# Superjie13/StereoTracking

Hardware: AMD Instinct MI355X
Metric: stereo frame-pairs/sec @1280x720 D=192 (higher is better)
Workload: dtype f32; 1 GPU; configs[1]: batch=8 synthetic 1280x720 stereo pairs per GPU, D=192, full YOLOX-s two-branch backbone+PAFPN+head, cost volume at 1/4 res (48 levels) + 2 3x3 aggregation convs + soft-argmin, decode+NMS, per-box depth; global_batch=8, inflight_contexts=4, distinct_input_batches=4, gpu_max_hw_queues=4, hip_force_dev_kernarg=1, parallelism=single process, no process group (no collective in the step), collectives_issued=0, tuning_plan=configs/tuning/mi355x.json, max_det=1000, detections_overflow=False

## Files before the change

include/stereotrack.h:

```cpp
#ifndef STEREOTRACK_H_
#define STEREOTRACK_H_

#include <stddef.h>
#include <stdint.h>

#ifdef __cplusplus
extern "C" {
#endif

#define ST_VERSION 430

enum {
  ST_OK = 0,
  ST_ERR_INVALID = -1,
  ST_ERR_HIP = -2,
  ST_ERR_STATE = -3,
  ST_ERR_WORKSPACE = -4,
  ST_ERR_NOTFOUND = -5
};

typedef void* st_stream_t;

int st_version(void);
const char* st_last_error(void);

typedef struct StConvDesc {
  const float* in_dev;
  int N, Hi, Wi, Cin, in_ld, in_off;
  const float* wgt_dev;
  const float* bias_dev;
  int Cout, KH, KW, stride, pad;
  float* out1_dev;
  int out1_ld, out1_off, split;
  float* out2_dev;
  int out2_ld, out2_off;
  float* up_dev;
  int up_ld, up_off;
  const float* res_dev;
  int res_ld, res_off;
  float post_scale;
  int act;
  const float* wgt_wino_dev;
} StConvDesc;

int st_conv2d_nhwc(const StConvDesc* d, st_stream_t stream);
int st_conv2d_nhwc_variant(const StConvDesc* d, st_stream_t stream, int variant);
size_t st_wino_packed_floats(int Cout, int Cin);
int st_wino_pack_weights(const float* packed_wgt_host, int Cout, int Cin, float* out_host);
int st_conv3x3_wino_group(const StConvDesc* descs, int n, st_stream_t stream);

int st_conv1x1_chain(const StConvDesc* a, const StConvDesc* b, st_stream_t stream);
size_t st_front_frag_floats(int Cout, int Cin);
int st_front_pack_frags(const float* packed_wgt_host, int Cout, int Cin, float* out_host);
int st_conv3x3s2_csp_front(const StConvDesc* a, const StConvDesc* ms, const StConvDesc* c1, const float* frag_ms_dev,
                           const float* frag_c1_dev, st_stream_t stream);
size_t st_csp_tail_frag_floats(void);
int st_csp_tail_pack_frags(const float* packed_wgt_host, float* out_host);
int st_conv3x3_csp_tail(const StConvDesc* conv2, const StConvDesc* fin, const float* frag_fin_dev, st_stream_t stream);
size_t st_conv_packed_floats(int Cout, int Cin, int KH, int KW);
int st_conv_pack_weights(const float* w, const float* conv_bias,
                         const float* bn_gamma, const float* bn_beta,
                         const float* bn_mean, const float* bn_var,
                         double bn_eps, int Cout, int Cin, int KH, int KW,
                         float* wgt_out, float* bias_out);

int st_focus_pack(const float* img_nchw_dev, int N, int C, int H, int W,
                  float* out_nhwc_dev, st_stream_t stream);

size_t st_stem_packed_floats(int Cout);
int st_stem_pack_weights(const float* w, const float* conv_bias,
                         const float* bn_gamma, const float* bn_beta,
                         const float* bn_mean, const float* bn_var,
                         double bn_eps, int Cout, int used_planes, float* wgt_out, float* bias_out);
int st_stem_focus_conv(const float* img_nchw_dev, int N, int H, int W, int used_planes, const float* wgt_dev,
                       const float* bias_dev, int Cout, float* out_nhwc_dev, int out_ld, int out_off,
                       int act , st_stream_t stream);
int st_stem_focus_conv_u8(const unsigned char* const* frames_u8_dev_ptrs_host, int N, int h, int w, int H, int W,
                          float pad_value, const float* wgt_dev, const float* bias_dev, int Cout, float* out_dev,
                          int out_ld, int out_off, int act, st_stream_t stream);

int st_pack_raw_inputs(const unsigned char* img_u8_dev, const unsigned short* disp_u16_dev, int N, int h, int w,
                       int H, int W, float img_pad, float* img_out_dev, float* disp_postp_out_dev,
                       float* disp_mask_out_dev, st_stream_t stream);
int st_pack_raw_frames(const unsigned char* const* frames_u8_dev_ptrs_host, int N, int h, int w, int H, int W,
                       float img_pad, float* img_out_dev, st_stream_t stream);
int st_resize_planes(const void* in_dev, int P, int h, int w, int interleaved, void* out_dev, int h2, int w2,
                     int elem_bytes, int bilinear, st_stream_t stream);

int st_spp_pool(const float* x_dev, int x_ld, int x_off, int N, int H, int W, int C,
                float* out_dev, int out_ld, int out_off, st_stream_t stream);

typedef struct StDetector StDetector;

typedef struct StDetectorConfig {
  int struct_size;
  float widen_factor;
  float deepen_factor;
  int num_classes;
  int batch;
  int height, width;
  double bn_eps;
  int with_right_branch;
  int disp_planes_identical;
  int rgb_only;
} StDetectorConfig;

int st_detector_create(const StDetectorConfig* cfg, StDetector** out);
int st_detector_destroy(StDetector* det);

int st_detector_num_params(const StDetector* det);
int st_detector_param_info(const StDetector* det, int idx, char* name, int name_cap,
                           int64_t shape[4], int* ndim);
int st_detector_set_param(StDetector* det, const char* name, const float* host, int64_t numel);
int st_detector_finalize(StDetector* det);

size_t st_detector_workspace_bytes(const StDetector* det);
size_t st_detector_head_floats(const StDetector* det);
int st_detector_num_levels(const StDetector* det);
int st_detector_level_info(const StDetector* det, int level, int* h, int* w, int* stride,
                           size_t* float_offset);
int st_detector_forward(StDetector* det, const float* img_dev, const float* disp_dev,
                        void* workspace_dev, size_t workspace_bytes, st_stream_t stream,
                        float* head_out_dev);
double st_detector_macs(const StDetector* det);
int st_detector_forward_phase(StDetector* det, int phase, const float* img_dev,
                              const float* disp_dev, const float* right_dev, void* workspace_dev,
                              size_t workspace_bytes, st_stream_t stream, float* head_out_dev);
int st_detector_forward_phase0_raw(StDetector* det, const unsigned char* const* left_frames_host,
                                   const unsigned char* const* right_frames_host, int h, int w, float pad_value,
                                   void* workspace_dev, size_t workspace_bytes, st_stream_t stream);
int st_detector_forward_raw(StDetector* det, const unsigned char* const* img_frames_host, int h, int w,
                            float pad_value, const float* disp_dev, void* workspace_dev, size_t workspace_bytes,
                            st_stream_t stream, float* head_out_dev);
int st_detector_set_timing(StDetector* det, int enable);
int st_detector_num_ops(const StDetector* det);
int st_detector_op_times(StDetector* det, int cap, float* ms, int* kind, int* variant, double* macs,
                         int* phase);
int st_detector_op_desc(const StDetector* det, int i, char* buf, int cap);
int st_detector_op_owner(const StDetector* det, int cap, int* owner, int* variant);
int st_split_instances_available(void);
int st_detector_set_split(StDetector* det, int allow);
int st_detector_autotune(StDetector* det, void* workspace_dev, size_t workspace_bytes,
                         float* head_out_dev, st_stream_t stream, int reps);
const char* st_conv_variant_name(int id);
const char* st_conv_variant_signature(int id);
int st_detector_get_tuning(const StDetector* det, int* variants, int cap);
int st_detector_set_tuning(StDetector* det, const int* variants, int n);
int st_detector_tap(const StDetector* det, const char* name, const void* workspace_dev,
                    const float** ptr_dev, int* N, int* C, int* H, int* W, int* ld);
typedef struct StHeadPredLevel {
  const float* cls_dev;
  int cls_ld, cls_off;
  const float* reg_dev;
  int reg_ld, reg_off;
  const float* wgt_cls_dev;
  const float* bias_cls_dev;
  const float* wgt_reg_dev;
  const float* bias_reg_dev;
  float* out_dev;
  int M;
} StHeadPredLevel;
int st_head_pred(const StHeadPredLevel levels[3], int feat, int num_classes, st_stream_t stream);

typedef struct StDecodeDesc {
  int struct_size;
  int batch;
  int num_levels;
  int level_h[4], level_w[4], level_stride[4];
  size_t level_offset[4];
  float score_thr;
  float iou_thr;
  int max_det;
  float scale_x, scale_y;
// ... 449 lines not shown
```

stereotracking_amd/_lib.py:

```python
import ctypes as C
import os

import torch

_HERE = os.path.dirname(os.path.abspath(__file__))
LIB_PATH = os.path.join(_HERE, 'lib', 'libstereotrack_hip.so')

ST_OK = 0
_ERR_NAMES = {-1: 'ST_ERR_INVALID', -2: 'ST_ERR_HIP', -3: 'ST_ERR_STATE', -4: 'ST_ERR_WORKSPACE',
              -5: 'ST_ERR_NOTFOUND'}


class StError(RuntimeError):
    """A libstereotrack_hip call returned a non-zero status."""


class StConvDesc(C.Structure):
    _fields_ = [
        ('in_dev', C.c_void_p),
        ('N', C.c_int), ('Hi', C.c_int), ('Wi', C.c_int), ('Cin', C.c_int), ('in_ld', C.c_int), ('in_off', C.c_int),
        ('wgt_dev', C.c_void_p), ('bias_dev', C.c_void_p),
        ('Cout', C.c_int), ('KH', C.c_int), ('KW', C.c_int), ('stride', C.c_int), ('pad', C.c_int),
        ('out1_dev', C.c_void_p), ('out1_ld', C.c_int), ('out1_off', C.c_int), ('split', C.c_int),
        ('out2_dev', C.c_void_p), ('out2_ld', C.c_int), ('out2_off', C.c_int),
# ... 116 lines not shown
class StMotChallengeArgs(C.Structure):
    _fields_ = [(n, C.c_int) for n in ('struct_size', 'num_frames', 'num_gt', 'num_pred', 'max_frame_objects', 'do_preproc',
                                       'num_distractors')] + [('distractors', C.c_int * 8), ('num_ws_cells', C.c_longlong)] + \
        [(n, C.c_void_p) for n in ('gt_rows', 'pred_rows', 'frame_gt_off', 'frame_pred_off', 'frame_ws_off', 'ws')] + \
        [('ws_bytes', C.c_size_t)] + [(n, C.c_void_p) for n in ('gt_keep', 'pred_keep', 'status')]


class StTrackletArgs(C.Structure):
    _fields_ = [(n, C.c_int) for n in ('struct_size', 'num_rows', 'num_out_rows', 'num_tracks', 'first', 'count',
                                       'num_groups', 'max_rows')] + \
        [(n, C.c_void_p) for n in ('rows', 'row_out_off', 'row_gap', 'trk_out_off', 'trk_order', 'trk_len_scale', 'ws')] + \
        [('ws_bytes', C.c_size_t), ('out_rows', C.c_void_p), ('status', C.c_void_p), ('phase_ticks', C.c_void_p)]


class StAflinkArgs(C.Structure):
    _fields_ = [(n, C.c_int) for n in ('struct_size', 'num_sets', 'num_tracks', 'num_rows', 'capacity', 'first', 'count',
                                       'chunk')] + \
        [(n, C.c_double) for n in ('t_lo', 't_hi', 'spatial_thr')] + \
        [(n, C.c_void_p) for n in ('feat', 'trk_off', 'trk_set', 'set_off', 'ws_off', 'ws_x', 'header', 'cand', 'conf',
                                   'logits')]


class StStreamTick(C.Structure):
    _fields_ = [('struct_size', C.c_int), ('streams', C.c_int), ('chunk', C.c_int), ('num_chunks', C.c_int),
                ('max_dets', C.c_int), ('det_rows', C.c_int), ('stream_of_slot', C.c_void_p), ('frame_ids', C.c_void_p)]


class StHeadPredLevel(C.Structure):
    _fields_ = [('cls_dev', C.c_void_p), ('cls_ld', C.c_int), ('cls_off', C.c_int),
                ('reg_dev', C.c_void_p), ('reg_ld', C.c_int), ('reg_off', C.c_int),
                ('wgt_cls_dev', C.c_void_p), ('bias_cls_dev', C.c_void_p),
                ('wgt_reg_dev', C.c_void_p), ('bias_reg_dev', C.c_void_p),
                ('out_dev', C.c_void_p), ('M', C.c_int)]


class StDecodeDesc(C.Structure):
    _fields_ = [
        ('struct_size', C.c_int), ('batch', C.c_int), ('num_levels', C.c_int),
        ('level_h', C.c_int * 4), ('level_w', C.c_int * 4), ('level_stride', C.c_int * 4),
        ('level_offset', C.c_size_t * 4),
        ('score_thr', C.c_float), ('iou_thr', C.c_float), ('max_det', C.c_int),
        ('scale_x', C.c_float), ('scale_y', C.c_float), ('pad_left', C.c_float), ('pad_top', C.c_float),
        ('ori_w', C.c_float), ('ori_h', C.c_float), ('nms_mask_rows', C.c_int), ('num_classes', C.c_int),
        ('single_label', C.c_int),
    ]


_vp, _i, _f, _sz = C.c_void_p, C.c_int, C.c_float, C.c_size_t
_PROTOS = {
    'st_version': (C.c_int, []),
    'st_head_row_floats': (_i, [_i]),
    'st_png_unfilter': (_i, [_vp, _i, _i, _i, _vp]),
    'st_stem_focus_conv_u8': (_i, [_vp, _i, _i, _i, _i, _i, _f, _vp, _vp, _i, _vp, _i, _i, _i, _vp]),
    'st_detector_forward_raw': (_i, [_vp, _vp, _i, _i, _f, _vp, _vp, _sz, _vp, _vp]),
    'st_detector_forward_phase0_raw': (_i, [_vp, _vp, _vp, _i, _i, _f, _vp, _sz, _vp]),
    'st_pack_raw_frames': (_i, [_vp, _i, _i, _i, _i, _i, _f, _vp, _vp]),
    'st_resize_planes': (_i, [_vp, _i, _i, _i, _i, _vp, _i, _i, _i, _i, _vp]),
    'st_detector_set_split': (_i, [_vp, _i]),
    'st_split_instances_available': (_i, []),
    'st_volume_agg3d': (_i, [_vp, _vp, _i, _i, _i, _i, _vp, _f, _i, _vp]),
    'st_last_error': (C.c_char_p, []),
    'st_conv2d_nhwc': (_i, [C.POINTER(StConvDesc), _vp]),
    'st_conv2d_nhwc_variant': (_i, [C.POINTER(StConvDesc), _vp, _i]),
    'st_conv3x3_wino_group': (_i, [C.POINTER(StConvDesc), _i, _vp]),
    'st_head_pred': (_i, [C.POINTER(StHeadPredLevel), _i, _i, _vp]),
    'st_detector_op_owner': (_i, [_vp, _i, _vp, _vp]),
    'st_conv1x1_chain': (_i, [C.POINTER(StConvDesc), C.POINTER(StConvDesc), _vp]),
    'st_front_frag_floats': (_sz, [_i, _i]),
    'st_front_pack_frags': (_i, [_vp, _i, _i, _vp]),
    'st_conv3x3s2_csp_front': (_i, [C.POINTER(StConvDesc), C.POINTER(StConvDesc), C.POINTER(StConvDesc), _vp, _vp, _vp]),
    'st_csp_tail_frag_floats': (_sz, []),
    'st_csp_tail_pack_frags': (_i, [_vp, _vp]),
    'st_conv3x3_csp_tail': (_i, [C.POINTER(StConvDesc), C.POINTER(StConvDesc), _vp, _vp]),
    'st_conv_packed_floats': (_sz, [_i, _i, _i, _i]),
    'st_wino_packed_floats': (_sz, [_i, _i]),
    'st_wino_pack_weights': (_i, [_vp, _i, _i, _vp]),
    'st_conv_pack_weights': (_i, [_vp, _vp, _vp, _vp, _vp, _vp, C.c_double, _i, _i, _i, _i, _vp, _vp]),
    'st_focus_pack': (_i, [_vp, _i, _i, _i, _i, _vp, _vp]),
    'st_stem_packed_floats': (_sz, [_i]),
    'st_stem_pack_weights': (_i, [_vp, _vp, _vp, _vp, _vp, _vp, C.c_double, _i, _i, _vp, _vp]),
    'st_stem_focus_conv': (_i, [_vp, _i, _i, _i, _i, _vp, _vp, _i, _vp, _i, _i, _i, _vp]),
    'st_pack_raw_inputs': (_i, [_vp, _vp, _i, _i, _i, _i, _i, _f, _vp, _vp, _vp, _vp]),
    'st_spp_pool': (_i, [_vp, _i, _i, _i, _i, _i, _i, _vp, _i, _i, _vp]),
    'st_detector_create': (_i, [C.POINTER(StDetectorConfig), C.POINTER(_vp)]),
    'st_detector_destroy': (_i, [_vp]),
    'st_detector_num_params': (_i, [_vp]),
    'st_detector_param_info': (_i, [_vp, _i, C.c_char_p, _i, C.POINTER(C.c_int64), C.POINTER(_i)]),
    'st_detector_set_param': (_i, [_vp, C.c_char_p, _vp, C.c_int64]),
    'st_detector_finalize': (_i, [_vp]),
    'st_detector_workspace_bytes': (_sz, [_vp]),
    'st_detector_head_floats': (_sz, [_vp]),
    'st_detector_num_levels': (_i, [_vp]),
    'st_detector_level_info': (_i, [_vp, _i, C.POINTER(_i), C.POINTER(_i), C.POINTER(_i), C.POINTER(_sz)]),
    'st_detector_forward': (_i, [_vp, _vp, _vp, _vp, _sz, _vp, _vp]),
    'st_detector_forward_phase': (_i, [_vp, _i, _vp, _vp, _vp, _vp, _sz, _vp, _vp]),
    'st_detector_macs': (C.c_double, [_vp]),
    'st_detector_set_timing': (_i, [_vp, _i]),
    'st_detector_num_ops': (_i, [_vp]),
    'st_detector_op_times': (_i, [_vp, _i, _vp, _vp, _vp, _vp, _vp]),
    'st_detector_autotune': (_i, [_vp, _vp, _sz, _vp, _vp, _i]),
    'st_conv_variant_name': (C.c_char_p, [_i]),
    'st_conv_variant_signature': (C.c_char_p, [_i]),
    'st_detector_get_tuning': (_i, [_vp, _vp, _i]),
    'st_detector_set_tuning': (_i, [_vp, _vp, _i]),
    'st_detector_op_desc': (_i, [_vp, _i, C.c_char_p, _i]),
    'st_detector_tap': (_i, [_vp, C.c_char_p, _vp, C.POINTER(_vp), C.POINTER(_i), C.POINTER(_i),
                             C.POINTER(_i), C.POINTER(_i), C.POINTER(_i)]),
    'st_decode_nms_workspace_bytes': (_sz, [C.POINTER(StDecodeDesc)]),
    'st_lapjv_extended': (_i, [_vp, _i, _i, C.c_double, _vp, _vp]),
    'st_tracker_create': (_i, [C.POINTER(StTrackerConfig), C.POINTER(_vp)]),
    'st_tracker_destroy': (_i, [_vp]),
    'st_tracker_reset': (_i, [_vp]),
    'st_tracker_track': (_i, [_vp, _i, _vp, _i, _vp, _vp, _i, C.POINTER(_i)]),
    'st_tracker_track_records': (_i, [_vp, _vp, _vp, _i, _i, _i, _vp, _vp, _i, _vp]),
    'st_tracker_cmc_needed': (_i, [_vp, _i, _i]),
    'st_tracker_track_cmc': (_i, [_vp, _i, _vp, _i, _vp, _vp, _vp, _i, C.POINTER(_i)]),
    'st_tracker_track_records_cmc': (_i, [_vp, _vp, _vp, _i, _i, _i, _vp, _vp, C.POINTER(_i), _vp, _vp, _i, _vp,
                                          C.POINTER(_i)]),
    'st_cmc_num_levels': (_i, [_vp]),
    'st_cmc_workspace_bytes': (_sz, [_i]),
    'st_cmc_front_u8': (_i, [_vp, _i, _i, _i, _i, _i, _vp, _vp]),
    'st_cmc_front_f32': (_i, [_vp, _i, _i, _i, _i, _i, _vp, _vp]),
    'st_cmc_flow': (_i, [_vp, _vp, _i, _i, _vp, _sz, _vp, _vp, _vp]),
    'st_cmc_estimate': (_i, [_vp, _vp, _i, _i, _i, C.POINTER(StCmcParams), _vp, _sz, _vp, _vp, _vp, _vp]),
    'st_cmc_mesh_fit': (_i, [_vp, _i, _i, _i, C.POINTER(StCmcParams), _vp, _sz, _vp, _vp, _vp, _vp]),
    'st_cmc_fit': (_i, [_vp, _i, _i, C.c_float, C.c_float, _vp, _sz, _vp, _vp, _vp]),
    'st_cmc_ecc_plane_size': (_i, [_i, _i, _i, C.POINTER(_i), C.POINTER(_i)]),
    'st_cmc_ecc_workspace_bytes': (_sz, [_i, _i, _i]),
    'st_cmc_ecc_front_u8': (_i, [_vp, _i, _i, _i, _i, _i, _i, _vp, _vp]),
    'st_cmc_ecc_front_f32': (_i, [_vp, _i, _i, _i, _i, _i, _i, _vp, _vp]),
    'st_cmc_ecc_prepare': (_i, [_vp, _vp, _i, _i, _i, C.POINTER(StEccParams), _vp, _sz, _vp, _vp, _vp, _vp, _vp]),
    'st_cmc_ecc_step': (_i, [_vp, _vp, _i, _i, _i, C.POINTER(StEccParams), _vp, _vp, _sz, _vp, _vp]),
    'st_cmc_ecc_estimate': (_i, [_vp, _vp, _i, _i, _i, C.POINTER(StEccParams), _vp, _sz, _vp, _vp, _vp]),
    'st_sgbm_workspace_bytes': (_sz, [_i, _i, _i, _i]),
    'st_sgbm_u8': (_i, [_vp, _vp, _i, _i, _i, _i, _i, C.POINTER(StSgbmParams), _vp, _sz, _vp, _i, _i, _vp, _vp]),
    'st_sgbm_f32': (_i, [_vp, _vp, _i, _i, _i, _i, _i, C.POINTER(StSgbmParams), _vp, _sz, _vp, _vp, _vp]),
    'st_sgbm_match_f32': (_i, [_vp, _vp, _i, _i, _i, _i, _i, C.POINTER(StSgbmParams), _vp, _sz, _vp, _vp, _vp]),
    'st_sgbm_median': (_i, [_vp, _i, _i, _i, _vp, _vp]),
    'st_sgbm_speckle': (_i, [_vp, _i, _i, _i, _i, _i, _vp, _sz, _vp, _vp, _i, _i, _vp, _vp]),
    'st_tracker_num_tracks': (_i, [_vp]),
    'st_tracker_next_id': (C.c_longlong, [_vp]),
    'st_tracker_get_track': (_i, [_vp, _i, _vp, _vp, _vp, C.POINTER(_i), C.POINTER(_i), C.POINTER(_i)]),
    'st_tracker_get_states': (_i, [_vp, _vp, _i, _i, C.POINTER(_i), C.POINTER(C.c_longlong)]),
    'st_batched_tracker_get_states': (_i, [_vp, _vp, _i, _vp, _i, _i, C.POINTER(_i), C.POINTER(C.c_longlong),
                                           C.POINTER(_i), _vp]),
    'st_batched_tracker_create': (_i, [C.POINTER(StTrackerConfig), _i, _i, _i, C.POINTER(_vp)]),
    'st_batched_tracker_create_multi': (_i, [C.POINTER(StTrackerConfig), _i, _i, _i, C.POINTER(_vp)]),
    'st_batched_tracker_run': (_i, [_vp, _vp, _vp, _vp, _vp, _i, _i, _i, _i, _vp, _vp, _vp, _vp, _vp, _vp, _vp]),
    'st_batched_tracker_destroy': (_i, [_vp]),
    'st_batched_tracker_state_bytes': (_sz, [_vp]),
    'st_batched_tracker_scratch_bytes': (_sz, [_vp]),
    'st_batched_tracker_step': (_i, [_vp, _vp, _vp, _vp, _vp, _vp, _vp, _vp, _vp, _vp, _vp]),
    'st_decode_nms': (_i, [C.POINTER(StDecodeDesc), _vp, _vp, _sz, _vp, _vp, _vp, _vp, _vp, _vp]),
    'st_costvolume_softargmin': (_i, [_vp, _vp, _i, _i, _i, _i, _i, _i, _f, _vp, _vp, _vp]),
    'st_softargmin': (_i, [_vp, _i, _i, _i, _i, _f, _vp, _vp]),
    'st_disp_upsample_pack': (_i, [_vp, _i, _i, _i, _i, _i, _i, _i, _i, _vp, _vp]),
    'st_softargmin_right': (_i, [_vp, _i, _i, _i, _i, _f, _vp, _vp]),
    'st_lr_check_pack': (_i, [_vp, _vp, _i, _i, _i, _i, _i, _i, _i, _i, _f, _vp, _vp, _vp]),
    'st_feat_upsample': (_i, [_vp, _i, _i, _i, _i, _i, _i, _vp, _vp]),
    'st_costvolume_agg3d_supported': (_i, [_i, _i]),
    'st_costvolume_agg3d': (_i, [_vp, _vp, _i, _i, _i, _i, _i, _i, _vp, _f, _i, _vp, _vp]),
    'st_costvolume_agg3d_softargmin': (_i, [_vp, _vp, _i, _i, _i, _i, _i, _i, _vp, _f, _i, _f, _vp, _vp]),
    'st_box_depth_workspace_bytes': (_sz, [_i, _i, _i, _i]),
    'st_pack_records': (_i, [_vp, _vp, _vp, _vp, _vp, _vp, _vp, _vp, _i, _i, _i, _i, _vp, _vp]),
    'st_box_depth': (_i, [_vp, _sz, _i, _i, _i, _vp, _vp, _i, _f, _f, _vp, _sz, _vp, _vp, _vp, _vp]),
    'st_coco_max_gt': (_i, []),
# ... 76 lines not shown
```

stereotracking_amd/csrc/detector.cpp:

```cpp
#include <algorithm>
#include <cmath>
#include <cstring>
#include <map>
#include <memory>
#include <vector>

#include "st_common.h"

namespace st {

int conv2d_launch(const StConvDesc& d, hipStream_t stream, int force_variant, int* picked_variant);
bool pw_conv_applicable(const StConvDesc& d);
bool pw_chain_applicable(const StConvDesc& d, const StConvDesc& c);
bool dc_conv_applicable(const StConvDesc& d);
bool wino_conv_applicable(const StConvDesc& d);
bool wino_shape_ok(int Cin, int Cout);
bool wino_group_applicable(const StConvDesc* d, int n);
int wino_group_launch(const StConvDesc* d, int n, hipStream_t stream);
size_t wino_packed_floats(int Cout, int Cin);
int wino_pack_weights(const float* packed, int Cout, int Cin, float* out);
int pw_conv_launch(const StConvDesc& d, hipStream_t stream, const StConvDesc* chain);
bool pwr_conv_applicable(const StConvDesc& d);
bool pwr_chain_applicable(const StConvDesc& d, const StConvDesc& c);
int pwr_conv_launch(const StConvDesc& d, hipStream_t stream, const StConvDesc* chain);
bool front_fused_applicable(const StConvDesc& a, const StConvDesc& ms, const StConvDesc& c1);
int front_fused_launch(const StConvDesc& a, const StConvDesc& ms, const StConvDesc& c1, const float* frag_ms_dev,
                       const float* frag_c1_dev, hipStream_t stream);
size_t front_frag_floats(int Cout, int Cin);
int front_pack_frags(const float* packed, int Cout, int Cin, float* out);
bool csp_tail_applicable(const StConvDesc& c2, const StConvDesc& f);
int csp_tail_launch(const StConvDesc& c2, const StConvDesc& f, const float* frag_fin_dev, hipStream_t stream);
size_t csp_tail_frag_floats();
int csp_tail_pack_frags(const float* packed, float* out);
int conv_variant_count();
bool conv_variant_valid(int id, int cout);
const char* conv_variant_name(int id);
const char* conv_variant_signature(int id);
int focus_pack_launch(const float* img, int N, int C, int H, int W, float* out, hipStream_t stream);
int stem_focus_conv_launch(const float* in, int N, int H, int W, int used_planes, const float* wgt,
                           const float* bias, int Cout, float* out, int out_ld, int out_off, int act,
                           hipStream_t stream, const StemRawInput* raw);
int spp_pool_launch(const float* x, int x_ld, int x_off, int N, int H, int W, int C, float* out,
                    int out_ld, int out_off, hipStream_t stream);
struct HeadPredLevel {
  const float *cls, *reg, *wc, *wr, *bc, *br;
  float* out;
  int cls_ld, cls_off, reg_ld, reg_off, M, blk0;
};
struct HeadPredArgs {
  HeadPredLevel lv[3];
  int Kpad, nc, nblocks;
};
bool head_pred_applicable(int feat, int nc);
int head_pred_launch(HeadPredArgs a, int feat, hipStream_t stream);

namespace {

int make_divisible(double x, double widen) { return (int)std::ceil(x * widen / 8.0) * 8; }
int make_round(int n, double deepen) {
  if (n <= 1) return n;
  const double v = n * deepen;
  double r = std::nearbyint(v);
  return std::max((int)r, 1);
}

struct Param {
  std::string name;
  std::vector<int64_t> shape;
  std::vector<float> data;
  bool set = false;
  int64_t numel() const {
    int64_t n = 1;
    for (auto s : shape) n *= s;
    return n;
  }
};

struct ConvSrc {
  std::string conv_prefix;
  std::string bn_prefix;
  bool has_bias;
  int cout;
};

struct PackedConv {
  std::vector<ConvSrc> srcs;
  int cin = 0, k = 1, cout = 0;
  size_t wgt_off = 0, bias_off = 0;
  size_t wino_off = 0;
  bool wino = false;
  size_t frag_off = 0;
  bool frag = false;
  size_t tail_off = 0;
  bool tail = false;
  bool stem = false;
  int stem_planes = 3;
};

constexpr int BUF_HEAD = -2;
constexpr int BUF_NONE = -1;

struct TRef {
  int buf = BUF_NONE;
  int N = 0, H = 0, W = 0, C = 0;
  int ld = 0, off = 0;
  size_t base = 0;
  bool adv = false;
  bool valid() const { return buf != BUF_NONE; }
  TRef slice(int o, int c) const {
    TRef t = *this;
    t.off = off + o;
    t.C = c;
    return t;
  }
};

struct Op {
  enum Type { FOCUS, CONV, SPP, STEM, PRED } type;
  int focus_input = 0;
  int focus_batch_off = 0;
  int pc = -1;
  TRef in, out1, out2, up, res;
  int split = 0, stride = 1, pad = 0, act = 1;
  float post_scale = 1.f;
  int phase = 0;
  double macs = 0.0;
// ... 491 lines not shown
                                    bn ? get(s.bn_prefix + ".weight") : nullptr, bn ? get(s.bn_prefix + ".bias") : nullptr,
                                    bn ? get(s.bn_prefix + ".running_mean") : nullptr,
                                    bn ? get(s.bn_prefix + ".running_var") : nullptr, det->cfg.bn_eps, s.cout, pc.cin,
                                    pc.k, pc.k, wtmp.data(), btmp.data()));
      std::memcpy(host.data() + pc.wgt_off + (size_t)row * Kpad, wtmp.data(), sizeof(float) * (size_t)s.cout * Kpad);
      std::memcpy(host.data() + pc.bias_off + row, btmp.data(), sizeof(float) * (size_t)s.cout);
      row += s.cout;
    }
    if (pc.wino) ST_CHECK(wino_pack_weights(host.data() + pc.wgt_off, pc.cout, pc.cin, host.data() + pc.wino_off));
    if (pc.frag) ST_CHECK(front_pack_frags(host.data() + pc.wgt_off, pc.cout, pc.cin, host.data() + pc.frag_off));
    if (pc.tail) ST_CHECK(csp_tail_pack_frags(host.data() + pc.wgt_off, host.data() + pc.tail_off));
  }
  if (!det->wgt_dev) ST_CHECK_HIP(hipMalloc(reinterpret_cast<void**>(&det->wgt_dev), det->wgt_floats * sizeof(float)));
  ST_CHECK_HIP(hipMemcpy(det->wgt_dev, host.data(), det->wgt_floats * sizeof(float), hipMemcpyHostToDevice));
  det->finalized = true;
  return ST_OK;
}

extern "C" size_t st_detector_workspace_bytes(const StDetector* det) { return det ? det->ws_floats * sizeof(float) : 0; }
extern "C" size_t st_detector_head_floats(const StDetector* det) { return det ? det->head_floats : 0; }
extern "C" int st_detector_num_levels(const StDetector* det) { return det ? det->n_levels : 0; }
extern "C" double st_detector_macs(const StDetector* det) { return det ? det->macs : 0.0; }

extern "C" int st_detector_level_info(const StDetector* det, int level, int* h, int* w, int* stride,
                                      size_t* float_offset) {
  if (!det || level < 0 || level >= det->n_levels) return set_error(ST_ERR_INVALID, "st_detector_level_info: bad level");
  if (h) *h = det->lvl_h[level];
  if (w) *w = det->lvl_w[level];
  if (stride) *stride = det->lvl_stride[level];
  if (float_offset) *float_offset = det->lvl_off[level];
  return ST_OK;
}

namespace {

float* resolve(const StDetector* det, const TRef& t, float* ws, float* head, int img0 = 0) {
  if (t.buf == BUF_NONE) return nullptr;
  if (t.buf == BUF_HEAD) return head + t.base;
  const size_t shift = t.adv ? (size_t)img0 * t.H * t.W * t.ld : 0;
  return ws + det->buf_off[t.buf] + t.base + shift;
}

StConvDesc conv_desc(const StDetector* det, const Op& o, int img0, float* ws, float* head) {
  const PackedConv& pc = det->convs[o.pc];
  StConvDesc d{};
  d.in_dev = resolve(det, o.in, ws, head, img0);
  d.N = o.in.N; d.Hi = o.in.H; d.Wi = o.in.W; d.Cin = pc.cin; d.in_ld = o.in.ld; d.in_off = o.in.off;
  d.wgt_dev = det->wgt_dev + pc.wgt_off;
  d.bias_dev = det->wgt_dev + pc.bias_off;
  d.Cout = pc.cout; d.KH = pc.k; d.KW = pc.k; d.stride = o.stride; d.pad = o.pad;
  d.out1_dev = resolve(det, o.out1, ws, head, img0); d.out1_ld = o.out1.ld; d.out1_off = o.out1.off;
  d.split = o.split;
  d.out2_dev = resolve(det, o.out2, ws, head, img0); d.out2_ld = o.out2.ld; d.out2_off = o.out2.off;
  d.up_dev = resolve(det, o.up, ws, head, img0); d.up_ld = o.up.ld; d.up_off = o.up.off;
  d.res_dev = resolve(det, o.res, ws, head, img0); d.res_ld = o.res.ld; d.res_off = o.res.off;
  d.post_scale = o.post_scale; d.act = o.act;
  d.wgt_wino_dev = pc.wino ? det->wgt_dev + pc.wino_off : nullptr;
  return d;
}

int launch_op(StDetector* det, Op& o, int img0, const float* const inputs[3], float* ws, float* head,
              hipStream_t stream) {
  switch (o.type) {
    case Op::FOCUS: {
      const float* src = inputs[o.focus_input];
      ST_REQUIRE(src != nullptr, "detector: input %d not provided (raw uint8 frames need the fused stem)", o.focus_input);
      float* dst = resolve(det, o.out1, ws, head) + (size_t)o.focus_batch_off * o.out1.H * o.out1.W * o.out1.ld;
      return focus_pack_launch(src, det->cfg.batch, 3, det->cfg.height, det->cfg.width, dst, stream);
    }
    case Op::STEM: {
      const float* src = inputs[o.focus_input];
      const StemRawInput* raw = det->raw_inputs[o.focus_input].frames ? &det->raw_inputs[o.focus_input] : nullptr;
      ST_REQUIRE(src != nullptr || raw != nullptr, "detector: input %d not provided", o.focus_input);
      const PackedConv& pc = det->convs[o.pc];
      float* dst = resolve(det, o.out1, ws, head) + (size_t)o.focus_batch_off * o.out1.H * o.out1.W * o.out1.ld;
      return stem_focus_conv_launch(src, det->cfg.batch, det->cfg.height, det->cfg.width, pc.stem_planes,
                                    det->wgt_dev + pc.wgt_off, det->wgt_dev + pc.bias_off, pc.cout, dst, o.out1.ld,
                                    o.out1.off, 1, stream, raw);
    }
    case Op::SPP: {
      float* x = resolve(det, o.in, ws, head, img0);
      float* out = resolve(det, o.out1, ws, head, img0);
      return spp_pool_launch(x, o.in.ld, o.in.off, o.in.N, o.in.H, o.in.W, o.in.C, out, o.out1.ld, o.out1.off,
                             stream);
    }
    case Op::PRED: {
      HeadPredArgs a{};
      for (int l = 0; l < 3; ++l) {
        const PackedConv &pcc = det->convs[o.pred_pcc[l]], &pcr = det->convs[o.pred_pcr[l]];
        HeadPredLevel& L = a.lv[l];
        L.cls = resolve(det, o.pred_cls[l], ws, head, img0); L.cls_ld = o.pred_cls[l].ld; L.cls_off = o.pred_cls[l].off;
        L.reg = resolve(det, o.pred_reg[l], ws, head, img0); L.reg_ld = o.pred_reg[l].ld; L.reg_off = o.pred_reg[l].off;
        L.wc = det->wgt_dev + pcc.wgt_off; L.bc = det->wgt_dev + pcc.bias_off;
        L.wr = det->wgt_dev + pcr.wgt_off; L.br = det->wgt_dev + pcr.bias_off;
        L.out = resolve(det, o.pred_out[l], ws, head, img0);
        L.M = o.pred_out[l].N * o.pred_out[l].H * o.pred_out[l].W;
        a.Kpad = round_up(pcc.cin, 32);
        a.nc = pcc.cout;
      }
      return head_pred_launch(a, det->convs[o.pred_pcc[0]].cin, stream);
    }
    case Op::CONV: {
      const PackedConv& pc = det->convs[o.pc];
      (void)pc;
      const StConvDesc d = conv_desc(det, o, img0, ws, head);
      return conv2d_launch(d, stream, det->force_variant >= 0 ? det->force_variant : o.tuned, &o.variant);
    }
  }
  return ST_OK;
}

int run_ops(StDetector* det, int phase_lo, int phase_hi, const float* const inputs[3], float* ws,
            float* head, hipStream_t stream) {
  const size_t ev_per_op = 2 * (size_t)det->max_group_count;
  if (det->timing && det->events.size() != ev_per_op * det->ops.size()) {
    for (auto& e : det->events) (void)hipEventDestroy(e);
    det->events.resize(ev_per_op * det->ops.size());
    for (auto& e : det->events) ST_CHECK_HIP(hipEventCreate(&e));
  }
  const size_t nops = det->ops.size();
  size_t oi = 0;
  while (oi < nops) {
    Op& first = det->ops[oi];
    if (first.phase < phase_lo || first.phase > phase_hi) { ++oi; continue; }
    size_t oe = oi + 1;
    if (first.group == 0 && first.wgroup > 0 && det->allow_wgroup && det->force_variant < 0) {
      size_t we = oi;
      StConvDesc wd[8];
      bool ok = true;
      while (we < nops && we - oi < 8 && det->ops[we].wgroup == first.wgroup && det->ops[we].phase == first.phase &&
             det->ops[we].group == 0) {
        const Op& o = det->ops[we];
        ok = ok && o.type == Op::CONV && (o.tuned == 43 || o.tuned == 44);
        if (ok) wd[we - oi] = conv_desc(det, o, 0, ws, head);
        ++we;
      }
      const int nw = (int)(we - oi);
#ifdef ST_ABLATION
      for (size_t k = oi; k < we; ++k) ok = ok && !(k < det->skip.size() && det->skip[k]);
#endif
      if (ok && nw >= 2 && wino_group_applicable(wd, nw)) {
        if (det->timing) ST_CHECK_HIP(hipEventRecord(det->events[ev_per_op * oi], stream));
        ST_CHECK(wino_group_launch(wd, nw, stream));
        for (size_t k = oi; k < we; ++k) {
          if (det->timing && k > oi) ST_CHECK_HIP(hipEventRecord(det->events[ev_per_op * k], stream));
          if (det->timing) ST_CHECK_HIP(hipEventRecord(det->events[ev_per_op * k + 1], stream));
          det->ops[k].variant = k == oi ? 48 : 49;
          det->ops[k].owner = (int)oi;
        }
        oi = we;
        continue;
      }
    }
    if (first.group > 0)
      while (oe < nops && det->ops[oe].group == first.group && det->ops[oe].phase == first.phase) ++oe;
    else if (first.chain_next && oe < nops && det->ops[oe].group == 0 && det->ops[oe].phase == first.phase)
      ++oe;
    const StDetector::Group g = det->groups[first.group];
    for (int sbi = 0; sbi < g.count; ++sbi) {
      int fused_left = 0, fused_variant = 0, fused_owner = -1;
      for (size_t k = oi; k < oe; ++k) {
        Op& o = det->ops[k];
        if (det->timing) ST_CHECK_HIP(hipEventRecord(det->events[ev_per_op * k + 2 * sbi], stream));
#ifdef ST_ABLATION
        const bool skipped = k < det->skip.size() && det->skip[k];
#else
        constexpr bool skipped = false;
// ... 361 lines not shown
```

stereotracking_amd/csrc/pack_pool.hip:

```cpp
#include <cstdint>
#include <algorithm>
#include <cstdlib>

#include "st_common.h"

namespace st {

typedef float f32x4 __attribute__((ext_vector_type(4)));
typedef float f32x2 __attribute__((ext_vector_type(2)));

template <int C>
__global__ __launch_bounds__(256) void focus_pack_kernel(const float* __restrict__ img, int N, int H,
                                                         int W, float* __restrict__ out) {
  const int Ho = H >> 1, Wo = W >> 1;
  const long long total = (long long)N * Ho * Wo;
  for (long long idx = (long long)blockIdx.x * blockDim.x + threadIdx.x; idx < total;
       idx += (long long)gridDim.x * blockDim.x) {
    const int ox = (int)(idx % Wo);
    const long long t = idx / Wo;
    const int oy = (int)(t % Ho);
    const int n = (int)(t / Ho);
    float v[4 * C];
#pragma unroll
    for (int c = 0; c < C; ++c) {
// ... 22 lines not shown
  const long long total = (long long)N * H * W * C4;
  for (long long idx = (long long)blockIdx.x * blockDim.x + threadIdx.x; idx < total;
       idx += (long long)gridDim.x * blockDim.x) {
    const int c4 = (int)(idx % C4);
    long long t = idx / C4;
    const int px = (int)(t % W);
    t /= W;
    const int py = (int)(t % H);
    const int n = (int)(t / H);
    const float ninf = -__builtin_inff();
    f32x4 m5 = {ninf, ninf, ninf, ninf}, m9 = m5, m13 = m5;
    for (int dy = -6; dy <= 6; ++dy) {
      const int yy = py + dy;
      if ((unsigned)yy >= (unsigned)H) continue;
      const int ady = dy < 0 ? -dy : dy;
      for (int dx = -6; dx <= 6; ++dx) {
        const int xx = px + dx;
        if ((unsigned)xx >= (unsigned)W) continue;
        const int adx = dx < 0 ? -dx : dx;
        const f32x4 v = *reinterpret_cast<const f32x4*>(
            x + ((size_t)(n * H + yy) * W + xx) * x_ld + x_off + 4 * c4);
        const int rad = ady > adx ? ady : adx;
#pragma unroll
        for (int e = 0; e < 4; ++e) {
          m13[e] = fmaxf(m13[e], v[e]);
          if (rad <= 4) m9[e] = fmaxf(m9[e], v[e]);
          if (rad <= 2) m5[e] = fmaxf(m5[e], v[e]);
        }
      }
    }
    float* o = out + ((size_t)(n * H + py) * W + px) * out_ld + out_off + 4 * c4;
    if (copy_x)
      *reinterpret_cast<f32x4*>(o) = *reinterpret_cast<const f32x4*>(
          x + ((size_t)(n * H + py) * W + px) * x_ld + x_off + 4 * c4);
    *reinterpret_cast<f32x4*>(o + C) = m5;
    *reinterpret_cast<f32x4*>(o + 2 * C) = m9;
    *reinterpret_cast<f32x4*>(o + 3 * C) = m13;
  }
}

template <int CG>
__global__ __launch_bounds__(256) void spp_pool_lds_kernel(const float* __restrict__ x, int x_ld, int x_off, int H,
                                                           int W, int C, float* __restrict__ out, int out_ld,
                                                           int out_off, int copy_x) {
  extern __shared__ __attribute__((aligned(16))) float sm[];
  const int HW = H * W, n = blockIdx.y, c0 = blockIdx.x * CG;
  float* A = sm;
  float* B = sm + HW * CG;
  const int total = HW * CG;
  for (int e = threadIdx.x; e < total; e += blockDim.x) {
    const int pix = e / CG, c = e - pix * CG;
    const float v = x[((size_t)n * HW + pix) * x_ld + x_off + c0 + c];
    A[e] = v;
    if (copy_x) out[((size_t)n * HW + pix) * out_ld + out_off + c0 + c] = v;
  }
  __syncthreads();
  for (int level = 1; level <= 3; ++level) {
    for (int e = threadIdx.x; e < total; e += blockDim.x) {
      const int pix = e / CG, c = e - pix * CG, py = pix / W, px = pix - py * W;
      float m = A[e];
#pragma unroll
      for (int d = 1; d <= 2; ++d) {
        if (px - d >= 0) m = fmaxf(m, A[(pix - d) * CG + c]);
        if (px + d < W) m = fmaxf(m, A[(pix + d) * CG + c]);
      }
      B[e] = m;
    }
    __syncthreads();
    for (int e = threadIdx.x; e < total; e += blockDim.x) {
      const int pix = e / CG, c = e - pix * CG, py = pix / W;
      float m = B[e];
#pragma unroll
      for (int d = 1; d <= 2; ++d) {
        if (py - d >= 0) m = fmaxf(m, B[(pix - d * W) * CG + c]);
        if (py + d < H) m = fmaxf(m, B[(pix + d * W) * CG + c]);
      }
      A[e] = m;
      out[((size_t)n * HW + pix) * out_ld + out_off + level * C + c0 + c] = m;
    }
    __syncthreads();
  }
}

int focus_pack_launch(const float* img, int N, int C, int H, int W, float* out, hipStream_t stream) {
  ST_REQUIRE(img && out, "focus_pack: null pointer");
  ST_REQUIRE(N > 0 && H > 0 && W > 0 && (H % 2) == 0 && (W % 2) == 0, "focus_pack: H, W must be even");
  const long long total = (long long)N * (H / 2) * (W / 2);
  const int blocks = (int)std::min<long long>((total + 255) / 256, 256 * 16);
  switch (C) {
    case 1: hipLaunchKernelGGL(focus_pack_kernel<1>, dim3(blocks), dim3(256), 0, stream, img, N, H, W, out); break;
    case 3: hipLaunchKernelGGL(focus_pack_kernel<3>, dim3(blocks), dim3(256), 0, stream, img, N, H, W, out); break;
    default: return set_error(ST_ERR_INVALID, "focus_pack: C must be 1 or 3 (got %d)", C);
  }
  ST_CHECK_HIP(hipGetLastError());
  return ST_OK;
}

int spp_pool_launch(const float* x, int x_ld, int x_off, int N, int H, int W, int C, float* out,
                    int out_ld, int out_off, hipStream_t stream) {
  ST_REQUIRE(x && out, "spp_pool: null pointer");
  ST_REQUIRE(C % 4 == 0 && x_ld % 4 == 0 && x_off % 4 == 0 && out_ld % 4 == 0 && out_off % 4 == 0,
             "spp_pool: channel counts/offsets must be multiples of 4");
  ST_REQUIRE(out_off + 4 * C <= out_ld && x_off + C <= x_ld, "spp_pool: slice exceeds ld");
  const int copy_x = !(x == out && x_ld == out_ld && x_off == out_off);
  int cg = 8;
  if ((long long)(C / 8) * N < 1024) cg = 4;
  const size_t lds = (size_t)2 * H * W * cg * sizeof(float);
  if (C % cg == 0 && lds <= 150 * 1024 && N <= 65535) {
    using Kern = void (*)(const float*, int, int, int, int, int, float*, int, int, int);
    const Kern kern = cg == 8 ? spp_pool_lds_kernel<8> : cg == 4 ? spp_pool_lds_kernel<4> : spp_pool_lds_kernel<2>;
    static bool attr_set[3] = {false, false, false};
    const int ai = cg == 8 ? 0 : cg == 4 ? 1 : 2;
    if (!attr_set[ai]) {
      ST_CHECK_HIP(hipFuncSetAttribute(reinterpret_cast<const void*>(kern), hipFuncAttributeMaxDynamicSharedMemorySize,
                                       150 * 1024));
      attr_set[ai] = true;
    }
    hipLaunchKernelGGL(kern, dim3(C / cg, N), dim3(256), lds, stream, x, x_ld, x_off, H, W, C, out, out_ld, out_off,
                       copy_x);
    ST_CHECK_HIP(hipGetLastError());
    return ST_OK;
  }
  const long long total = (long long)N * H * W * (C / 4);
  const int blocks = (int)std::min<long long>((total + 255) / 256, 256 * 16);
  hipLaunchKernelGGL(spp_pool_kernel, dim3(blocks), dim3(256), 0, stream, x, x_ld, x_off, N, H, W, C,
                     out, out_ld, out_off, copy_x);
  ST_CHECK_HIP(hipGetLastError());
  return ST_OK;
}

}

extern "C" int st_focus_pack(const float* img, int N, int C, int H, int W, float* out,
                             st_stream_t stream) {
  return st::focus_pack_launch(img, N, C, H, W, out, static_cast<hipStream_t>(stream));
}

extern "C" int st_spp_pool(const float* x, int x_ld, int x_off, int N, int H, int W, int C,
                           float* out, int out_ld, int out_off, st_stream_t stream) {
  return st::spp_pool_launch(x, x_ld, x_off, N, H, W, C, out, out_ld, out_off,
                             static_cast<hipStream_t>(stream));
}

namespace st {

__global__ __launch_bounds__(256) void pack_raw_inputs_kernel(const unsigned char* __restrict__ img,
                                                              const unsigned short* __restrict__ disp, int N, int h,
                                                              int w, int H, int W, float img_pad,
                                                              float* __restrict__ img_out,
                                                              float* __restrict__ disp_out,
                                                              float* __restrict__ mask_out) {
  const long long total = (long long)N * H * W;
  for (long long idx = (long long)blockIdx.x * blockDim.x + threadIdx.x; idx < total;
       idx += (long long)gridDim.x * blockDim.x) {
    const int X = (int)(idx % W);
    const long long t = idx / W;
    const int Y = (int)(t % H);
    const int n = (int)(t / H);
    const bool inside = Y < h && X < w;
    const size_t plane = (size_t)H * W;
    if (img_out) {
#pragma unroll
      for (int c = 0; c < 3; ++c) {
        const float v = inside ? (float)img[(((size_t)n * 3 + c) * h + Y) * w + X] : img_pad;
        img_out[((size_t)n * 3 + c) * plane + (size_t)Y * W + X] = v;
      }
    }
    if (disp_out) {
      float d = 0.f, m = 0.f;
      if (inside) {
        const unsigned code = disp[((size_t)n * h + Y) * w + X];
        m = code < 65535u ? 1.f : 0.f;
        d = (code == 65535u ? 0.f : (float)code) / 16.0f;
      }
#pragma unroll
      for (int c = 0; c < 3; ++c) disp_out[((size_t)n * 3 + c) * plane + (size_t)Y * W + X] = d;
      if (mask_out) mask_out[(size_t)n * plane + (size_t)Y * W + X] = m;
    }
  }
}


__global__ __launch_bounds__(256) void pack_raw_inputs_vec4_kernel(const unsigned char* __restrict__ img,
                                                                   const unsigned short* __restrict__ disp, int N,
                                                                   int h, int w, int H, int W, float img_pad,
                                                                   float* __restrict__ img_out,
                                                                   float* __restrict__ disp_out,
                                                                   float* __restrict__ mask_out) {
  const int W4 = W >> 2;
  const long long total = (long long)N * H * W4;
  const size_t plane = (size_t)H * W;
  for (long long idx = (long long)blockIdx.x * blockDim.x + threadIdx.x; idx < total;
       idx += (long long)gridDim.x * blockDim.x) {
    const int X = (int)(idx % W4) << 2;
    const long long t = idx / W4;
    const int Y = (int)(t % H);
    const int n = (int)(t / H);
    const bool inside = Y < h && X < w;
    if (img_out) {
#pragma unroll
      for (int c = 0; c < 3; ++c) {
        float4 v = make_float4(img_pad, img_pad, img_pad, img_pad);
        if (inside) {
          const uchar4 q = *reinterpret_cast<const uchar4*>(img + (((size_t)n * 3 + c) * h + Y) * w + X);
          v = make_float4((float)q.x, (float)q.y, (float)q.z, (float)q.w);
        }
        *reinterpret_cast<float4*>(img_out + ((size_t)n * 3 + c) * plane + (size_t)Y * W + X) = v;
      }
    }
    if (disp_out) {
      float4 d = make_float4(0.f, 0.f, 0.f, 0.f), m = d;
      if (inside) {
        const ushort4 q = *reinterpret_cast<const ushort4*>(disp + ((size_t)n * h + Y) * w + X);
        const unsigned code[4] = {q.x, q.y, q.z, q.w};
        float dv[4], mv[4];
#pragma unroll
        for (int k = 0; k < 4; ++k) {
          mv[k] = code[k] < 65535u ? 1.f : 0.f;
          dv[k] = (code[k] == 65535u ? 0.f : (float)code[k]) / 16.0f;
        }
        d = make_float4(dv[0], dv[1], dv[2], dv[3]);
        m = make_float4(mv[0], mv[1], mv[2], mv[3]);
      }
// ... 178 lines not shown
```

Before: 1833 stereo frame-pairs/s.

## Add cascaded 5x5 max-pool SPP kernel with LDS ping-pong as default

```diff
diff --git a/include/stereotrack.h b/include/stereotrack.h
--- a/include/stereotrack.h
+++ b/include/stereotrack.h
@@ -89,6 +89,11 @@
 
 int st_spp_pool(const float* x_dev, int x_ld, int x_off, int N, int H, int W, int C,
                 float* out_dev, int out_ld, int out_off, st_stream_t stream);
+#define ST_SPP_AUTO 0
+#define ST_SPP_SWEEPS 1
+#define ST_SPP_CASCADE 2
+int st_spp_pool_form(const float* x_dev, int x_ld, int x_off, int N, int H, int W, int C,
+                     float* out_dev, int out_ld, int out_off, int form, st_stream_t stream);
 
 typedef struct StDetector StDetector;
 
diff --git a/stereotracking_amd/_lib.py b/stereotracking_amd/_lib.py
--- a/stereotracking_amd/_lib.py
+++ b/stereotracking_amd/_lib.py
@@ -222,6 +222,7 @@
     'st_stem_focus_conv': (_i, [_vp, _i, _i, _i, _i, _vp, _vp, _i, _vp, _i, _i, _i, _vp]),
     'st_pack_raw_inputs': (_i, [_vp, _vp, _i, _i, _i, _i, _i, _f, _vp, _vp, _vp, _vp]),
     'st_spp_pool': (_i, [_vp, _i, _i, _i, _i, _i, _i, _vp, _i, _i, _vp]),
+    'st_spp_pool_form': (_i, [_vp, _i, _i, _i, _i, _i, _i, _vp, _i, _i, _i, _vp]),
     'st_detector_create': (_i, [C.POINTER(StDetectorConfig), C.POINTER(_vp)]),
     'st_detector_destroy': (_i, [_vp]),
     'st_detector_num_params': (_i, [_vp]),
diff --git a/stereotracking_amd/csrc/detector.cpp b/stereotracking_amd/csrc/detector.cpp
--- a/stereotracking_amd/csrc/detector.cpp
+++ b/stereotracking_amd/csrc/detector.cpp
@@ -41,7 +41,7 @@
                            const float* bias, int Cout, float* out, int out_ld, int out_off, int act,
                            hipStream_t stream, const StemRawInput* raw);
 int spp_pool_launch(const float* x, int x_ld, int x_off, int N, int H, int W, int C, float* out,
-                    int out_ld, int out_off, hipStream_t stream);
+                    int out_ld, int out_off, int form, hipStream_t stream);
 struct HeadPredLevel {
   const float *cls, *reg, *wc, *wr, *bc, *br;
   float* out;
@@ -699,7 +699,7 @@
       float* x = resolve(det, o.in, ws, head, img0);
       float* out = resolve(det, o.out1, ws, head, img0);
       return spp_pool_launch(x, o.in.ld, o.in.off, o.in.N, o.in.H, o.in.W, o.in.C, out, o.out1.ld, o.out1.off,
-                             stream);
+                             ST_SPP_AUTO, stream);
     }
     case Op::PRED: {
       HeadPredArgs a{};
diff --git a/stereotracking_amd/csrc/pack_pool.hip b/stereotracking_amd/csrc/pack_pool.hip
--- a/stereotracking_amd/csrc/pack_pool.hip
+++ b/stereotracking_amd/csrc/pack_pool.hip
@@ -128,6 +128,69 @@
   }
 }
 
+__device__ __forceinline__ f32x4 max4(const f32x4 a, const f32x4 b) {
+  return f32x4{fmaxf(a[0], b[0]), fmaxf(a[1], b[1]), fmaxf(a[2], b[2]), fmaxf(a[3], b[3])};
+}
+
+template <int CG>
+__global__ __launch_bounds__(1024) void spp_cascade_kernel(const float* __restrict__ x, int x_ld, int x_off, int H,
+                                                           int W, int C, float* __restrict__ out, int out_ld,
+                                                           int out_off, int copy_x, int seg, int nseg) {
+  extern __shared__ __attribute__((aligned(16))) float sm[];
+  constexpr int NQ = CG / 4;
+  const int HW = H * W, cols = W * NQ, total = HW * NQ;
+  const int tid = threadIdx.x, nthr = blockDim.x;
+  const float* xin = x + (size_t)blockIdx.y * HW * x_ld + x_off + blockIdx.x * CG;
+  float* o = out + (size_t)blockIdx.y * HW * out_ld + out_off + blockIdx.x * CG;
+  f32x4* src = reinterpret_cast<f32x4*>(sm);
+  f32x4* dst = src + total;
+  for (int e0 = tid; e0 < total; e0 += 4 * nthr) {
+    f32x4 v[4];
+#pragma unroll
+    for (int k = 0; k < 4; ++k) {
+      const int e = e0 + k * nthr, pix = e / NQ, q = e - pix * NQ;
+      if (e < total) v[k] = *reinterpret_cast<const f32x4*>(xin + (size_t)pix * x_ld + 4 * q);
+    }
+#pragma unroll
+    for (int k = 0; k < 4; ++k) {
+      const int e = e0 + k * nthr, pix = e / NQ, q = e - pix * NQ;
+      if (e < total) {
+        src[e] = v[k];
+        if (copy_x) *reinterpret_cast<f32x4*>(o + (size_t)pix * out_ld + 4 * q) = v[k];
+      }
+    }
+  }
+  __syncthreads();
+  const float ninf = -__builtin_inff();
+  const f32x4 ninf4 = {ninf, ninf, ninf, ninf};
+  for (int level = 1; level <= 3; ++level) {
+    for (int it = tid; it < cols * nseg; it += nthr) {
+      const int s = it / cols, col = it - s * cols, px = col / NQ, q = col - px * NQ;
+      const int y0 = s * seg, y1 = min(y0 + seg, H);
+      int tap[5];
+#pragma unroll
+      for (int d = 0; d < 5; ++d) tap[d] = min(max(px + d - 2, 0), W - 1) * NQ + q;
+      f32x4 w0 = ninf4, w1 = ninf4, w2 = ninf4, w3 = ninf4;
+      for (int yy = y0 - 2; yy < y1 + 2; ++yy) {
+        f32x4 r = ninf4;
+        if ((unsigned)yy < (unsigned)H) {
+          const f32x4* row = src + yy * cols;
+          r = max4(max4(max4(row[tap[0]], row[tap[1]]), max4(row[tap[2]], row[tap[3]])), row[tap[4]]);
+        }
+        const f32x4 m = max4(max4(max4(w0, w1), max4(w2, w3)), r);
+        w0 = w1; w1 = w2; w2 = w3; w3 = r;
+        const int y = yy - 2;
+        if (y >= y0) {
+          if (level < 3) dst[y * cols + col] = m;
+          *reinterpret_cast<f32x4*>(o + (size_t)(y * W + px) * out_ld + level * C + 4 * q) = m;
+        }
+      }
+    }
+    if (level < 3) __syncthreads();
+    f32x4* t = src; src = dst; dst = t;
+  }
+}
+
 int focus_pack_launch(const float* img, int N, int C, int H, int W, float* out, hipStream_t stream) {
   ST_REQUIRE(img && out, "focus_pack: null pointer");
   ST_REQUIRE(N > 0 && H > 0 && W > 0 && (H % 2) == 0 && (W % 2) == 0, "focus_pack: H, W must be even");
@@ -143,12 +206,45 @@
 }
 
 int spp_pool_launch(const float* x, int x_ld, int x_off, int N, int H, int W, int C, float* out,
-                    int out_ld, int out_off, hipStream_t stream) {
+                    int out_ld, int out_off, int form, hipStream_t stream) {
   ST_REQUIRE(x && out, "spp_pool: null pointer");
   ST_REQUIRE(C % 4 == 0 && x_ld % 4 == 0 && x_off % 4 == 0 && out_ld % 4 == 0 && out_off % 4 == 0,
              "spp_pool: channel counts/offsets must be multiples of 4");
   ST_REQUIRE(out_off + 4 * C <= out_ld && x_off + C <= x_ld, "spp_pool: slice exceeds ld");
+  ST_REQUIRE(N > 0 && H > 0 && W > 0 && C > 0, "spp_pool: bad geometry");
+  ST_REQUIRE(form == ST_SPP_AUTO || form == ST_SPP_SWEEPS || form == ST_SPP_CASCADE, "spp_pool: unknown form %d", form);
   const int copy_x = !(x == out && x_ld == out_ld && x_off == out_off);
+  if (form != ST_SPP_SWEEPS) {
+    int ccg = 16, threads = 1024;
+#ifdef ST_ABLATION
+    if (const char* e = getenv("ST_SPP_CG")) ccg = atoi(e) == 8 ? 8 : 16;
+    if (const char* e = getenv("ST_SPP_THREADS")) threads = atoi(e) == 512 ? 512 : atoi(e) == 256 ? 256 : 1024;
+#endif
+    const size_t clds = (size_t)2 * H * W * ccg * sizeof(float);
+    const bool aligned = ((reinterpret_cast<uintptr_t>(x) | reinterpret_cast<uintptr_t>(out)) & 15) == 0;
+    if (C % ccg == 0 && clds <= 150 * 1024 && N <= 65535 && aligned) {
+      const int cols = W * (ccg / 4);
+      const int want = std::min(std::max(threads / cols, 1), H);
+      const int seg = (H + want - 1) / want, nseg = (H + seg - 1) / seg;
+      static int lds_set[2] = {0, 0};
+#ifdef ST_ABLATION
+      if (ccg == 8) {
+        ST_ENSURE_DYNAMIC_LDS(spp_cascade_kernel<8>, clds, lds_set[1]);
+        hipLaunchKernelGGL(spp_cascade_kernel<8>, dim3(C / 8, N), dim3(threads), clds, stream, x, x_ld, x_off, H, W, C,
+                           out, out_ld, out_off, copy_x, seg, nseg);
+      } else
+#endif
+      {
+        ST_ENSURE_DYNAMIC_LDS(spp_cascade_kernel<16>, clds, lds_set[0]);
+        hipLaunchKernelGGL(spp_cascade_kernel<16>, dim3(C / 16, N), dim3(threads), clds, stream, x, x_ld, x_off, H, W, C,
+                           out, out_ld, out_off, copy_x, seg, nseg);
+      }
+      ST_CHECK_HIP(hipGetLastError());
+      return ST_OK;
+    }
+    ST_REQUIRE(form != ST_SPP_CASCADE, "spp_pool: the cascade kernel needs C %% 16 == 0, 16-byte aligned buffers and "
+               "2 x H x W x 16 floats <= 150 KB of LDS");
+  }
   int cg = 8;
   if ((long long)(C / 8) * N < 1024) cg = 4;
   const size_t lds = (size_t)2 * H * W * cg * sizeof(float);
@@ -184,7 +280,13 @@
 
 extern "C" int st_spp_pool(const float* x, int x_ld, int x_off, int N, int H, int W, int C,
                            float* out, int out_ld, int out_off, st_stream_t stream) {
-  return st::spp_pool_launch(x, x_ld, x_off, N, H, W, C, out, out_ld, out_off,
+  return st::spp_pool_launch(x, x_ld, x_off, N, H, W, C, out, out_ld, out_off, ST_SPP_AUTO,
+                             static_cast<hipStream_t>(stream));
+}
+
+extern "C" int st_spp_pool_form(const float* x, int x_ld, int x_off, int N, int H, int W, int C,
+                                float* out, int out_ld, int out_off, int form, st_stream_t stream) {
+  return st::spp_pool_launch(x, x_ld, x_off, N, H, W, C, out, out_ld, out_off, form,
                              static_cast<hipStream_t>(stream));
 }
 
```

After: 1841 stereo frame-pairs/s, median of 6. No clear change (+0.4%).
